# jaehyuck0103/OpenMAVIS

Measured on AMD Instinct MI355X. Metric: multi-cam frames/sec (ORB extract+match) + LocalBA iters/sec, 5x720x540, higher is better.
Workload: dtype u8

## Files before the change

### openmavis_amd/csrc/orb_extract.hip

```cpp
#include <hip/hip_runtime.h>

#include <algorithm>
#include <cmath>
#include <cstdlib>
#include <climits>
#include <cstdio>
#include <cstring>
#include <vector>

#include "../../include/omv.h"
#include "fast_plan.h"
#include "omv_device.h"
#include "omv_host.h"
#include "omv_introsort.h"

namespace {

constexpr int kMaxLevels = 16;
constexpr int kOrbStages = 4;
using omv_fast_plan::kEdge;
using omv_fast_plan::kMinB;
#define OMV_PATTERN_TABLE_BEGIN
#define OMV_PATTERN_TABLE_END
constexpr int kPattern[256 * 4] = {
#include "orb_pattern_31.inc"
};
struct FloatPattern {
    float v[256][4];
};
constexpr FloatPattern float_pattern() {
    FloatPattern p{};
    for (int i = 0; i < 256; ++i)
        for (int q = 0; q < 4; ++q) p.v[i][q] = (float)kPattern[4 * i + q];
    return p;
}
__constant__ FloatPattern c_patternf = float_pattern();
__constant__ int c_gauss7[7] = {18, 34, 48, 56, 48, 34, 18};

struct LevelGeom {
    int w, h, pitch;
    long long off;
    int maxBX, maxBY;
    int cell_begin, cell_end;
    int quota;
    int out_cap;
    int out_off;
    long long cand_off;
    int cand_cap;
    int nIni;
    float hX;
    float scale;
    float size;
    int xtab_off, ytab_off;
    int xq_off, use_xq;
    uint32_t m_quads, m_groups, m_w;
};

using omv_fast_plan::Cell;
using omv_fast_plan::FastSlot;

struct Geom {
    int nlevels;
    int W, H;
// ... 298 lines not shown

typedef _Float16 h2 __attribute__((ext_vector_type(2)));
__device__ __forceinline__ h2 h2_swap(h2 x) { return h2{x.y, x.x}; }
typedef unsigned short u16x2 __attribute__((ext_vector_type(2)));
__device__ __forceinline__ h2 h2_bytes(const uint8_t *lo, const uint8_t *hi) {
    const u16x2 v{(unsigned short)*lo, (unsigned short)*hi};
    return __builtin_bit_cast(h2, v);
}

template <int RS>
__device__ __forceinline__ int fast_strength_h(const uint8_t *p7, int stride_rt) {
    const int stride = RS > 0 ? RS : stride_rt;
    const int c = 3 * stride + 3;
    const int o[16] = {c + 3 * stride, c + 3 * stride + 1, c + 2 * stride + 2, c + stride + 3, c + 3, c - stride + 3,
                       c - 2 * stride + 2, c - 3 * stride + 1, c - 3 * stride, c - 3 * stride - 1, c - 2 * stride - 2,
                       c - stride - 3, c - 3, c + stride - 3, c + 2 * stride - 2, c + 3 * stride - 1};
    const h2 vv = h2_bytes(p7 + c, p7 + c);
    h2 d[8];
#pragma unroll
    for (int k = 0; k < 8; ++k) d[k] = vv - h2_bytes(p7 + o[k], p7 + o[k + 8]);
    auto Q = [&](const h2 *a, int k) { return k < 8 ? a[k] : h2_swap(a[k - 8]); };
    h2 t3n[8], t3x[8];
#pragma unroll
    for (int k = 0; k < 8; ++k) {
        t3n[k] = __builtin_elementwise_minimum(__builtin_elementwise_minimum(d[k], Q(d, k + 1)), Q(d, k + 2));
        t3x[k] = __builtin_elementwise_maximum(__builtin_elementwise_maximum(d[k], Q(d, k + 1)), Q(d, k + 2));
    }
    h2 a{(_Float16)-1000, (_Float16)-1000}, b{(_Float16)1000, (_Float16)1000};
#pragma unroll
    for (int k = 0; k < 8; ++k) {
        const h2 m9 = __builtin_elementwise_minimum(__builtin_elementwise_minimum(t3n[k], Q(t3n, k + 3)), Q(t3n, k + 6));
        const h2 M9 = __builtin_elementwise_maximum(__builtin_elementwise_maximum(t3x[k], Q(t3x, k + 3)), Q(t3x, k + 6));
        a = __builtin_elementwise_maximum(a, m9);
        b = __builtin_elementwise_minimum(b, M9);
    }
    const pk16 m = __builtin_elementwise_max(__builtin_bit_cast(pk16, a),
                                             __builtin_bit_cast(pk16, __builtin_bit_cast(uint32_t, b) ^ 0x80008000u));
    return max(max((int)m.x, (int)m.y), 0);
}

__device__ __forceinline__ int wave_incl_scan_dpp(int v) {
    v += __builtin_amdgcn_update_dpp(0, v, 0x111, 0xf, 0xf, false);
    v += __builtin_amdgcn_update_dpp(0, v, 0x112, 0xf, 0xf, false);
    v += __builtin_amdgcn_update_dpp(0, v, 0x114, 0xf, 0xf, false);
    v += __builtin_amdgcn_update_dpp(0, v, 0x118, 0xf, 0xf, false);
    v += __builtin_amdgcn_update_dpp(0, v, 0x142, 0xa, 0xf, false);
    v += __builtin_amdgcn_update_dpp(0, v, 0x143, 0xc, 0xf, false);
    return v;
}

#ifdef OMV_FAST_PROFILE
__device__ unsigned long long g_fast_stats[8];
#endif
template <int RS>
__global__ void __launch_bounds__(64) fast_cells_kernel(Geom g, const Cell *cells, const FastSlot *slots,
                                                        const uint8_t *images, size_t img_stride, size_t pitch0,
                                                        const uint8_t *pyr, int *cell_cnt, uint32_t *cell_kp, int rmax,
                                                        int smax, int n_blocks) {
    extern __shared__ __attribute__((aligned(16))) uint8_t smem[];
    const int blk = omv::xcd_block(n_blocks);
    if (blk < 0) return;
    const int img = blk / g.n_cells;
    const int ci = blk - img * g.n_cells;
    const Cell c = cells[ci];
    const int lane = threadIdx.x;
    const FastSlot sl0 = slots[c.slot_off + lane];
    const int rw = c.x1 - c.x0, rh = c.y1 - c.y0;
    int sp;
    const uint8_t *src = level_base(g, images, img_stride, pitch0, pyr, img, c.level, &sp);
    const uint8_t *row0 = src + (size_t)c.y0 * sp + c.x0;
    const bool dwords = ((sp & 3) == 0) && ((((uintptr_t)src) & 3) == 0);
    const int o = dwords ? c.o : 0;
    const int rs = RS > 0 ? RS : dwords ? 4 * c.nd : ((rw + 3) & ~3);
    uint8_t *pix = smem + o;
    uint8_t *S = smem + rmax;
    const int sw = rw - 4;
    uint16_t *cand = (uint16_t *)(smem + rmax + smax);
    if (dwords) {
        const int nd = c.nd;
        const uint8_t *g0 = row0 - o;
        uint32_t *l0 = (uint32_t *)smem;
        const int rpi = c.rpi, lr = omv::mul_u24(lane, (int)c.mnd) >> 16, w = lane - omv::mul_u24(lr, nd);
        if (lr < rpi) {
            uint32_t gs = (uint32_t)(omv::mul_u24(lr, sp) + 4 * w);
            uint32_t *ld = l0 + omv::mul_u24(lr, rs >> 2) + w;
            const uint32_t gstep = (uint32_t)(rpi * sp);
            const int lstep = rpi * (rs >> 2);
#pragma unroll 4
            for (int b = 0; b < c.nband; ++b, gs += gstep, ld += lstep) *ld = *(const uint32_t *)(g0 + gs);
            if (lr < rh - c.nband * rpi) *ld = *(const uint32_t *)(g0 + gs);
        }
    } else {
        for (int i = lane; i < rw * rh; i += 64) {
            const int r = i / rw, q = i - r * rw;
            pix[r * rs + q] = row0[(size_t)r * sp + q];
        }
    }
    for (int i = lane; i < (sw * (rh - 4) + 15) >> 4; i += 64) ((uint4 *)S)[i] = make_uint4(0, 0, 0, 0);
    __syncthreads();
    const int dw = rw - 6, dh = rh - 6;
    const int ndet = c.ndet;
    const uint32_t mdw = c.mdw;
    auto rowcol = [&](int i, int &r, int &q) {
        const int rr = omv::mul_u24(i, (int)mdw) >> 20;
        r = 3 + rr, q = 3 + i - omv::mul_u24(rr, dw);
    };
    const uint64_t lt = (1ull << lane) - 1ull;
#ifdef OMV_FAST_PROFILE
    int ncand_last = 0;
#endif
    auto prefilter = [&](int t) {
        int ncand = 0;
        if (dwords && ndet > 0) {
            const int rsw = rs >> 2;
            const int np = c.np;
            const pk16 T0{(short)t, (short)t};
            auto lo = [](uint32_t a, uint32_t b, uint32_t s) {
                return __builtin_bit_cast(pk16, __builtin_amdgcn_perm(a, b, 0x0c000c00u | ((s + 1) << 16) | s));
            };
            auto hi = [](uint32_t a, uint32_t b, uint32_t s) {
                return __builtin_bit_cast(pk16, __builtin_amdgcn_perm(a, b, 0x0c000c00u | ((s + 3) << 16) | (s + 2)));
            };
            auto test = [&](pk16 v, pk16 n0, pk16 n4, pk16 n8, pk16 n12) {
                const pk16 vp = v + T0, vm = v - T0;
                auto sg = [](pk16 x) { return __builtin_bit_cast(uint32_t, x); };
                const pk16 hi = __builtin_elementwise_min(__builtin_elementwise_max(n0, n8), __builtin_elementwise_max(n4, n12));
                const pk16 lo = __builtin_elementwise_max(__builtin_elementwise_min(n0, n8), __builtin_elementwise_min(n4, n12));
                return (sg(vp - hi) | sg(lo - vm)) & 0x80008000u;
            };
            auto compass = [&](uint32_t up) {
                const uint32_t *wu = reinterpret_cast<const uint32_t *>(smem + up);
                const uint32_t U0 = wu[0], U1 = wu[1];
                const uint32_t Wm = wu[3 * rsw - 1], C0 = wu[3 * rsw], C1 = wu[3 * rsw + 1], Wp = wu[3 * rsw + 2];
                const uint32_t D0 = wu[6 * rsw], D1 = wu[6 * rsw + 1];
                const uint32_t p0 = test(lo(C0, C0, 0), lo(D0, D0, 0), lo(C1, C0, 3), lo(U0, U0, 0), lo(C0, Wm, 1));
                const uint32_t p1 = test(hi(C0, C0, 0), hi(D0, D0, 0), hi(C1, C0, 3), hi(U0, U0, 0), hi(C0, Wm, 1));
                const uint32_t p2 = test(lo(C1, C1, 0), lo(D1, D1, 0), lo(Wp, C1, 3), lo(U1, U1, 0), lo(C1, C0, 1));
                const uint32_t p3 = test(hi(C1, C1, 0), hi(D1, D1, 0), hi(Wp, C1, 3), hi(U1, U1, 0), hi(C1, C0, 1));
                const uint32_t xb = (p0 >> 15) | (p1 >> 13) | (p2 >> 11) | (p3 >> 9);
                return (xb & 0x55u) | ((xb >> 15) & 0xaau);
            };
            const uint32_t lpos0 = (uint32_t)(rmax + smax);
            uint32_t lpos = lpos0;
            const uint8_t *sl = reinterpret_cast<const uint8_t *>(slots + c.slot_off);
            const uint32_t sl_lane = (uint32_t)lane * (uint32_t)sizeof(FastSlot);
            FastSlot nx = sl0;
            for (int t0 = 0; t0 < np; t0 += 64) {
                const FastSlot cur = nx;
                nx = *reinterpret_cast<const FastSlot *>(sl + (size_t)(t0 + 64) * sizeof(FastSlot) + sl_lane);
                uint32_t bits = compass(cur.hi) & (cur.lo >> 16);
                const int cnt = __popc(bits);
                const int incl = wave_incl_scan_dpp(cnt);
                if (bits) {
                    uint16_t *cp = reinterpret_cast<uint16_t *>(smem + lpos + 2u * (uint32_t)(incl - cnt)) - 1;
                    const uint32_t ebase = cur.lo & 0xffffu;
                    uint32_t below = bits - 1u;
                    for (;;) {
                        *++cp = (uint16_t)(ebase + __builtin_ctz(bits));
                        bits &= below;
                        if (__builtin_usub_overflow(bits, 1u, &below)) break;
                    }
                }
                lpos += 2u * (uint32_t)__builtin_amdgcn_readlane(incl, 63);
            }
            ncand = (int)((lpos - lpos0) >> 1);
        } else {
            for (int i0 = 0; i0 < ndet; i0 += 64) {
                const int i = i0 + lane;
                bool pass = false;
                int r = 0, q = 0;
                if (i < ndet) {
                    rowcol(i, r, q);
                    const uint8_t *p = pix + r * rs + q;
                    const int v = p[0];
                    const int d0 = v - p[3 * rs], d4 = v - p[3], d8 = v - p[-3 * rs], d12 = v - p[-3];
                    const bool a0 = d0 > t, a4 = d4 > t, a8 = d8 > t, a12 = d12 > t;
                    const bool b0 = d0 < -t, b4 = d4 < -t, b8 = d8 < -t, b12 = d12 < -t;
                    pass = (a0 && a4) || (a4 && a8) || (a8 && a12) || (a12 && a0) || (b0 && b4) || (b4 && b8) ||
                           (b8 && b12) || (b12 && b0);
                }
                const uint64_t m = __ballot(pass);
                if (pass) cand[ncand + __popcll(m & lt)] = (uint16_t)((r << 7) | q);
                ncand += __popcll(m);
            }
        }
        __syncthreads();
#ifdef OMV_FAST_PROFILE
        ncand_last = ncand;
#endif
        const uint8_t *pix7 = smem + __builtin_amdgcn_readfirstlane(o - (3 * rs + 3));
        int ncorn = 0;
        for (int k0 = 0; k0 < ncand; k0 += 64) {
            const int k = k0 + lane;
            bool corner = false;
            int e = 0;
            if (k < ncand) {
                e = cand[k];
                const int r = e >> 7, q = e & 127;
                const int sv = fast_strength_h<RS>(pix7 + r * rs + q, rs);
                S[omv::mul_u24(r - 2, sw) + (q - 2)] = (uint8_t)sv;
                corner = sv > t;
            }
            const uint64_t m = __ballot(corner);
            if (corner) cand[ncorn + __popcll(m & lt)] = (uint16_t)e;
            ncorn += __popcll(m);
        }
        __syncthreads();
        return ncorn;
    };
    auto nms = [&](int ncorn, int th, uint32_t *out) {
        int base = 0;
        for (int k0 = 0; k0 < ncorn; k0 += 64) {
            const int k = k0 + lane;
            bool keep = false;
            uint32_t packed = 0;
            if (k < ncorn) {
                const int e = cand[k];
                const int r = e >> 7, q = e & 127;
                const uint8_t *sp8 = S + omv::mul_u24(r - 2, sw) + (q - 2);
                const int v = sp8[0];
                int m = max(th, 1);
#pragma unroll
                for (int n = 0; n < 9; ++n)
                    if (n != 4) m = max(m, (int)sp8[(n / 3 - 1) * sw + (n % 3 - 1)]);
                keep = v > m;
                const int x = c.x0 + q - kMinB, y = c.y0 + r - kMinB;
                packed = (uint32_t)x | ((uint32_t)y << 12) | ((uint32_t)(v - 1) << 24);
            }
            const uint64_t m = __ballot(keep);
            const int pos = base + __popcll(m & lt);
            if (out && keep && pos < g.cell_cap) out[pos] = packed;
            base += __popcll(m);
        }
        return base;
    };
    uint32_t *out = cell_kp + (size_t)blk * g.cell_cap;
    int th = g.ini_th;
    int ncorn = prefilter(th);
#ifdef OMV_FAST_PROFILE
    const int ncand0 = ncand_last;
#endif
    int total = nms(ncorn, th, out);
    if (total == 0) {
        th = g.min_th;
        ncorn = prefilter(th);
        total = nms(ncorn, th, out);
    }
    if (lane == 0) cell_cnt[blk] = total > g.cell_cap ? -1 : total;
#ifdef OMV_FAST_PROFILE
    {
        __shared__ int dummy;
        (void)dummy;
        if (lane == 0) {
            atomicAdd(&g_fast_stats[0], 1ull);
            atomicAdd(&g_fast_stats[1], (unsigned long long)ndet);
            atomicAdd(&g_fast_stats[2], (unsigned long long)ncand0);
            atomicAdd(&g_fast_stats[3], th == g.min_th && g.min_th != g.ini_th ? 1ull : 0ull);
            atomicAdd(&g_fast_stats[4], (unsigned long long)ncand_last);
            atomicAdd(&g_fast_stats[5], (unsigned long long)total);
            atomicAdd(&g_fast_stats[6], (unsigned long long)ncorn);
            __threadfence();
            const unsigned long long done = atomicAdd(&g_fast_stats[7], 1ull) + 1;
            if (done == (unsigned long long)n_blocks)
                printf("fast: cells %llu pixels %llu cand(iniTh) %llu retries %llu cand(last pass) %llu corners(last pass) "
                       "%llu keypoints %llu\n",
                       g_fast_stats[0], g_fast_stats[1], g_fast_stats[2], g_fast_stats[3], g_fast_stats[4],
                       g_fast_stats[6], g_fast_stats[5]);
        }
    }
#endif
}

__device__ __forceinline__ int wave_incl_scan(int v) { return wave_incl_scan_dpp(v); }

__device__ int block_excl_scan(int *a, int n, int *tmp) {
    const int tid = threadIdx.x, T = blockDim.x;
    const int chunk = (n + T - 1) / T;
    const int b = min(n, tid * chunk), e = min(n, b + chunk);
    int s = 0;
    for (int i = b; i < e; ++i) s += a[i];
    const int incl = wave_incl_scan(s);
    const int wave = tid >> 6, nw = T >> 6;
    __syncthreads();
    if ((tid & 63) == 63) tmp[wave] = incl;
    __syncthreads();
    int woff = 0, tot = 0;
    for (int w = 0; w < nw; ++w) {
        if (w < wave) woff += tmp[w];
        tot += tmp[w];
    }
    int run = woff + incl - s;
    for (int i = b; i < e; ++i) {
        const int v = a[i];
        a[i] = run;
        run += v;
    }
    __syncthreads();
    return tot;
}

__device__ int2 block_excl_scan2(int *a, int na, int *b, int nb, int *tmp) {
    const int tid = threadIdx.x, T = blockDim.x;
    const int ca = (na + T - 1) / T, a0 = min(na, tid * ca), a1 = min(na, a0 + ca);
    const int cb = (nb + T - 1) / T, b0 = min(nb, tid * cb), b1 = min(nb, b0 + cb);
    int sa = 0, sb = 0;
    for (int i = a0; i < a1; ++i) sa += a[i];
    for (int i = b0; i < b1; ++i) sb += b[i];
    const int ia = wave_incl_scan(sa), ib = wave_incl_scan(sb);
    const int wave = tid >> 6, nw = T >> 6;
    __syncthreads();
    if ((tid & 63) == 63) tmp[wave] = ia, tmp[8 + wave] = ib;
    __syncthreads();
    int oa = 0, ta = 0, ob = 0, tb = 0;
    for (int w = 0; w < nw; ++w) {
        if (w < wave) oa += tmp[w], ob += tmp[8 + w];
        ta += tmp[w], tb += tmp[8 + w];
    }
    int run = oa + ia - sa;
    for (int i = a0; i < a1; ++i) {
        const int v = a[i];
        a[i] = run;
        run += v;
    }
// ... 583 lines not shown
    }
    const int rank = (int)(cl & 0x7fffffffu);
    const int row = (cl >> 31) ? total - 1 - (lap_before + rank) : mono_before + rank;
    omv_kp *kp = a.kps + (size_t)img * g.n_max + row;
    uint64_t *dst = reinterpret_cast<uint64_t *>(a.desc + ((size_t)img * g.n_max + row) * 32);
    if (lane < 4) dst[lane] = words[lane];
    if (a.harris && lane == 0) a.harris[(size_t)img * g.n_max + row] = harris;
    if (lane == 0) {
        float x = (float)cx, y = (float)cy;
        if (l != 0) x *= L.scale, y *= L.scale;
        *kp = omv_kp{x, y, L.size, angle, (float)score, l};
    }
}

inline int host_round_even(float v) { return (int)std::nearbyint(v); }

__global__ void __launch_bounds__(256) node_sort_selftest_kernel(const int *k1, const int *k2, int n, int *perm) {
    extern __shared__ __attribute__((aligned(16))) int ssm[];
    omv::SortItem *items = reinterpret_cast<omv::SortItem *>(ssm);
    omv::SortItem *tmp = items + n;
    int *LS = reinterpret_cast<int *>(tmp + n), *RS = LS + n, *stk = RS + n;
    for (int i = threadIdx.x; i < n; i += blockDim.x) items[i] = omv::SortItem{k1[i], k2[i], i};
    __syncthreads();
    omv::block_introsort_loop(items, n, stk, LS, RS, threadIdx.x, blockDim.x);
    omv::block_final_insertion_sort(items, n, tmp, threadIdx.x, blockDim.x);
    for (int i = threadIdx.x; i < n; i += blockDim.x) perm[i] = items[i].payload;
}

}

struct omv_orb {
    omv_orb_params p;
    int W, H, max_images;
    int pyr_mode = -1;
    std::vector<float> scale, inv_scale, sigma2, inv_sigma2;
    std::vector<int> quota;
    int umax[16];
    Geom g;
    Cell *d_cells = nullptr;
    FastSlot *d_slots = nullptr;
    XTab *d_xt = nullptr, *d_yt = nullptr;
    XQuad *d_xq = nullptr;
    uint32_t *d_disc = nullptr;
    uint64_t *d_bop = nullptr;
    float *harris = nullptr;
    uint8_t *d_pyr = nullptr;
    int *d_cell_cnt = nullptr;
    uint32_t *d_cell_kp = nullptr, *d_cand = nullptr, *d_nid = nullptr, *d_lvl_out = nullptr, *d_lvl_cls = nullptr;
    int *d_lvl_cnt = nullptr, *d_lap = nullptr, *d_err = nullptr;
    int rmax = 0;
    int smax = 0;
    int fast_rs = 0;
    size_t fast_lds = 0;
    size_t oct_lds = 0;
    size_t pyr_lds[kMaxLevels] = {};
    PyrBand *d_bands = nullptr;
    int pyr_nb = 0, pyr_buf_dw = 0;
    int pyr_tab_dw = 0, pyr_rows = 0;
    int pyr_ydw = 3;
    uint8_t *d_img1 = nullptr;
    omv_kp *d_kp1 = nullptr;
    uint8_t *d_desc1 = nullptr;
    int *d_n1 = nullptr;
    std::vector<int> h_lap;
    hipStream_t last_stream = nullptr;
    int last_n = 0;
    int device = 0;
    bool timing = false;
    std::vector<hipEvent_t> ev;
    double stage_ms[kOrbStages] = {};
    long long stage_calls = 0;
    omv::DeviceArena mem;
    ~omv_orb() { for (hipEvent_t e : ev) (void)hipEventDestroy(e); }
};

static void flush_timing(omv_orb *o) {
    for (size_t b = 0; b + kOrbStages + 1 <= o->ev.size(); b += kOrbStages + 1) {
        for (int k = 0; k < kOrbStages; ++k) {
            float ms = 0.f;
            (void)hipEventElapsedTime(&ms, o->ev[b + k], o->ev[b + k + 1]);
            o->stage_ms[k] += ms;
        }
        o->stage_calls++;
    }
    for (hipEvent_t e : o->ev) (void)hipEventDestroy(e);
    o->ev.clear();
}

static void mark(omv_orb *o, hipStream_t st) {
    if (!o->timing) return;
    hipEvent_t e;
    (void)hipEventCreate(&e);
    (void)hipEventRecord(e, st);
    o->ev.push_back(e);
}

static omv_status build_geometry(omv_orb *o, std::vector<Cell> &cells, std::vector<FastSlot> &slots, std::vector<XTab> &xt,
                                  std::vector<XTab> &yt, std::vector<XQuad> &xq) {
    const omv_orb_params &p = o->p;
    const int nl = p.nlevels;
    const double sf = (double)p.scale_factor;
    o->scale.assign(nl, 1.f), o->sigma2.assign(nl, 1.f), o->inv_scale.resize(nl), o->inv_sigma2.resize(nl);
    for (int i = 1; i < nl; ++i) {
        o->scale[i] = (float)(o->scale[i - 1] * sf);
        o->sigma2[i] = o->scale[i] * o->scale[i];
    }
// ... 228 lines not shown
            }
            return worst;
        };
        std::vector<PyrBand> bands;
        for (int budget : {8192, 16384}) {
            for (int nb = 8; nb <= 128 && L > 1 && !o->pyr_nb; ++nb) {
                const int worst = plan(nb, bands);
                if (worst > budget) continue;
                int tab = 0, rows = 0, ydw = 3;
                for (int l = 1; l < L; ++l) {
                    if (g.lv[l].use_xq) ydw = 4;
                    else tab = std::max(tab, 3 * g.lv[l].w);
                    for (int b = 0; b < nb; ++b) {
                        const PyrBand &pb = bands[(size_t)b * kMaxLevels + l];
                        rows = std::max(rows, pb.need_hi - pb.need_lo);
                    }
                }
                o->pyr_nb = nb, o->pyr_buf_dw = worst, o->pyr_tab_dw = (tab + 3) & ~3, o->pyr_rows = rows, o->pyr_ydw = ydw;
                if (!mem.alloc(&o->d_bands, bands.size())) return OMV_ERR_HIP;
                HIP_OK(hipMemcpy(o->d_bands, bands.data(), sizeof(PyrBand) * bands.size(), hipMemcpyHostToDevice));
                const int lds = (int)(sizeof(uint32_t) * (2 * (size_t)worst + 4 + o->pyr_tab_dw + (size_t)ydw * rows));
                if (lds > 160 * 1024) {
                    (void)mem.free(&o->d_bands);
                    o->pyr_nb = 0;
                    break;
                }
                if (lds > 64 * 1024)
                    (void)hipFuncSetAttribute((const void *)pyr_chain_kernel, hipFuncAttributeMaxDynamicSharedMemorySize, lds);
            }
        }
    }
    if (!mem.alloc(&o->d_xt, xt.size()) || !mem.alloc(&o->d_yt, yt.size())) return OMV_ERR_HIP;
    if (!xt.empty()) HIP_OK(hipMemcpy(o->d_xt, xt.data(), sizeof(XTab) * xt.size(), hipMemcpyHostToDevice));
    if (!yt.empty()) HIP_OK(hipMemcpy(o->d_yt, yt.data(), sizeof(XTab) * yt.size(), hipMemcpyHostToDevice));
    if (!mem.alloc(&o->d_xq, xq.size())) return OMV_ERR_HIP;
    if (!xq.empty()) HIP_OK(hipMemcpy(o->d_xq, xq.data(), sizeof(XQuad) * xq.size(), hipMemcpyHostToDevice));
    {
        const std::vector<uint32_t> dt = disc_table(o->umax);
        uint64_t bop[4 * 64];
        omv_fast_plan::describe_bop_table(bop);
        static_assert(64 * 8 * sizeof(uint32_t) % sizeof(uint64_t) == 0, "the operands follow the masks, 8-byte aligned");
        if (!mem.alloc(&o->d_disc, dt.size() + sizeof(bop) / sizeof(uint32_t))) return OMV_ERR_HIP;
        o->d_bop = reinterpret_cast<uint64_t *>(o->d_disc + dt.size());
        HIP_OK(hipMemcpy(o->d_disc, dt.data(), sizeof(uint32_t) * dt.size(), hipMemcpyHostToDevice));
        HIP_OK(hipMemcpy(o->d_bop, bop, sizeof(bop), hipMemcpyHostToDevice));
    }
    if (!mem.alloc(&o->d_pyr, std::max<size_t>(256, (size_t)g.pyr_bytes * n)) ||
        !mem.alloc(&o->d_cell_cnt, (size_t)g.n_cells * n) || !mem.alloc(&o->d_cell_kp, (size_t)g.n_cells * g.cell_cap * n) ||
        !mem.alloc(&o->d_cand, (size_t)g.cand_per_img * n) || !mem.alloc(&o->d_nid, (size_t)g.cand_per_img * n) ||
        !mem.alloc(&o->d_lvl_out, (size_t)g.out_per_img * n) || !mem.alloc(&o->d_lvl_cls, (size_t)g.out_per_img * n) ||
        !mem.alloc(&o->d_lvl_cnt, (size_t)3 * g.nlevels * n) || !mem.alloc(&o->d_lap, 2 * n) || !mem.alloc(&o->d_err, 1))
        return OMV_ERR_HIP;
    HIP_OK(hipMemset(o->d_err, 0, sizeof(int)));
    *out = owner.release();
    return OMV_OK;
}

omv_status omv_orb_destroy(omv_orb *o) {
    if (!o) return OMV_ERR_ARG;
    delete o;
    return OMV_OK;
}

int omv_orb_max_keypoints(const omv_orb *o) { return o ? o->g.n_max : 0; }

omv_status omv_orb_scale_tables(const omv_orb *o, float *scale, float *inv_scale, float *sigma2, float *inv_sigma2) {
    if (!o) return OMV_ERR_ARG;
    for (int l = 0; l < o->p.nlevels; ++l) {
        if (scale) scale[l] = o->scale[l];
        if (inv_scale) inv_scale[l] = o->inv_scale[l];
        if (sigma2) sigma2[l] = o->sigma2[l];
        if (inv_sigma2) inv_sigma2[l] = o->inv_sigma2[l];
    }
    return OMV_OK;
}

omv_status omv_orb_extract_batch(omv_orb *o, int n, const uint8_t *images, size_t image_stride, size_t pitch,
                                 const int *lapping, omv_kp *kps, uint8_t *desc, int *n_out, int *mono_index,
                                 void *stream) {
    if (!o || n <= 0 || n > o->max_images || !images || !lapping || !kps || !desc || !n_out || !mono_index)
        return OMV_ERR_ARG;
    if (pitch < (size_t)o->W || image_stride < pitch * o->H) return OMV_ERR_ARG;
    if (pitch >= ((size_t)1 << 24)) return OMV_ERR_ARG;
    hipStream_t st = (hipStream_t)stream;
    o->last_stream = st;
    o->last_n = n;
    const Geom &g = o->g;
    if (o->h_lap.size() < (size_t)2 * n || std::memcmp(o->h_lap.data(), lapping, sizeof(int) * 2 * n) != 0) {
        HIP_OK(hipMemcpyAsync(o->d_lap, lapping, sizeof(int) * 2 * n, hipMemcpyHostToDevice, st));
        o->h_lap.assign(lapping, lapping + 2 * n);
    }
    mark(o, st);
    const bool chain = o->pyr_mode >= 0 ? o->pyr_mode == 1 : n <= kPyrChainMaxImages;
    if (o->pyr_nb > 0 && chain) {
        const size_t lds = sizeof(uint32_t) * (2 * (size_t)o->pyr_buf_dw + 4 + o->pyr_tab_dw + (size_t)o->pyr_ydw * o->pyr_rows);
        pyr_chain_kernel<<<dim3(o->pyr_nb, n), 256, lds, st>>>(g, images, image_stride, pitch, o->d_pyr, o->d_xt, o->d_yt,
                                                               o->d_xq, o->d_bands, o->pyr_buf_dw, o->pyr_tab_dw);
    } else {
        for (int l = 1; l < g.nlevels; ++l) {
            pyr_resize_kernel<<<dim3((g.lv[l].h + kPyrBlock - 1) / kPyrBlock, n), 256, o->pyr_lds[l], st>>>(
                g, l, images, image_stride, pitch, o->d_pyr, o->d_xt, o->d_yt, o->d_xq, n);
        }
    }
    mark(o, st);
    if (o->fast_rs == 52)
        fast_cells_kernel<52><<<omv::xcd_grid(g.n_cells * n), 64, o->fast_lds, st>>>(
            g, o->d_cells, o->d_slots, images, image_stride, pitch, o->d_pyr, o->d_cell_cnt, o->d_cell_kp, o->rmax, o->smax,
            g.n_cells * n);
    else if (o->fast_rs == 68)
        fast_cells_kernel<68><<<omv::xcd_grid(g.n_cells * n), 64, o->fast_lds, st>>>(
            g, o->d_cells, o->d_slots, images, image_stride, pitch, o->d_pyr, o->d_cell_cnt, o->d_cell_kp, o->rmax, o->smax,
            g.n_cells * n);
    else
        fast_cells_kernel<0><<<omv::xcd_grid(g.n_cells * n), 64, o->fast_lds, st>>>(
            g, o->d_cells, o->d_slots, images, image_stride, pitch, o->d_pyr, o->d_cell_cnt, o->d_cell_kp, o->rmax, o->smax,
            g.n_cells * n);
    mark(o, st);
    OctArgs oa{o->d_cell_cnt, o->d_cell_kp, o->d_cand, o->d_nid, o->d_lvl_out, o->d_lvl_cls, o->d_lvl_cnt, o->d_lap, o->d_err};
    if (n <= kOctSmallImages) octree_kernel<1><<<g.nlevels * n, 256, o->oct_lds, st>>>(g, oa);
    else octree_kernel<OMV_OCT_WGS><<<g.nlevels * n, 256, o->oct_lds, st>>>(g, oa);
    mark(o, st);
    DescArgs da{images, image_stride, pitch, o->d_pyr, o->d_lvl_out, o->d_lvl_cls, o->d_lvl_cnt, kps, desc, n_out, mono_index, n,
                o->d_disc, o->harris, o->d_bop};
    const int waves = g.out_per_img * n;
    describe_kernel<<<omv::xcd_grid((waves + 3) / 4), 256, 0, st>>>(g, da, (waves + 3) / 4);
    mark(o, st);
    HIP_OK(hipGetLastError());
    return OMV_OK;
}

omv_status omv_orb_set_harris(omv_orb *o, float *harris) {
    if (!o) return OMV_ERR_ARG;
    o->harris = harris;
    return OMV_OK;
}

omv_status omv_orb_enable_timing(omv_orb *o, int on) {
    if (!o) return OMV_ERR_ARG;
    o->timing = on != 0;
    return OMV_OK;
}

omv_status omv_orb_stage_ms(omv_orb *o, double *ms4, long long *calls, int reset) {
    if (!o || !ms4) return OMV_ERR_ARG;
    HIP_OK(hipStreamSynchronize(o->last_stream));
    flush_timing(o);
    for (int k = 0; k < kOrbStages; ++k) ms4[k] = o->stage_ms[k];
    if (calls) *calls = o->stage_calls;
    if (reset) {
        for (int k = 0; k < kOrbStages; ++k) o->stage_ms[k] = 0;
        o->stage_calls = 0;
    }
    return OMV_OK;
}

omv_status omv_orb_last_error(omv_orb *o) {
    if (!o) return OMV_ERR_ARG;
    HIP_OK(hipStreamSynchronize(o->last_stream));
    int e = 0;
    HIP_OK(hipMemcpy(&e, o->d_err, sizeof(int), hipMemcpyDeviceToHost));
    HIP_OK(hipMemset(o->d_err, 0, sizeof(int)));
    return e;
}

omv_status omv_orb_extract_host(omv_orb *o, const uint8_t *image, size_t pitch, int lap0, int lap1, omv_kp *kps,
                                uint8_t *desc, int *n_out, int *mono_index) {
    if (!o || !image || !kps || !desc || !n_out || !mono_index) return OMV_ERR_ARG;
    const size_t dp = (size_t)o->W;
    if (!o->d_n1) {
// ... 61 lines not shown
```

Baseline: 53730.

## Make FAST cell kernel persistent with per-XCD atomic claims and register prefetch

Replaces the one-block-per-cell FAST launch with a persistent grid sized to occupancy. Each block claims batches of cells from per-XCD atomic counters and prefetches the next cell's pixel rows and slot data into registers while the current cell is processed. A last-block-exits counter resets the claim counters for the next launch. The intent is to hide global-load latency and cut block launch overhead, at the cost of heavy register use (up to 16 prefetch words, waves_per_eu hint), atomic contention and more complex control flow.

```diff
diff --git a/openmavis_amd/csrc/fast_claims.h b/openmavis_amd/csrc/fast_claims.h
--- /dev/null
+++ b/openmavis_amd/csrc/fast_claims.h
@@ -0,0 +1,37 @@
+#pragma once
+
+#if defined(__HIPCC__)
+#define OMV_CLAIM_FN __host__ __device__ inline
+#else
+#define OMV_CLAIM_FN inline
+#endif
+
+namespace omv_fast_claims {
+
+constexpr int kXcds = 8;
+constexpr int kCounterStride = 1024;
+constexpr int kMaxBatch = 4;
+constexpr int kExitCounter = kXcds * kCounterStride;
+constexpr int kClaimWords = kExitCounter + kCounterStride;
+
+OMV_CLAIM_FN int claim_block(int xcd, unsigned k, int j, int batch, int n) {
+    const unsigned chunk = (unsigned)(n + kXcds - 1) / kXcds;
+    const unsigned i = k * (unsigned)batch + (unsigned)j;
+    const unsigned b = (unsigned)xcd * chunk + i;
+    return (j < batch && i < chunk && b < (unsigned)n) ? (int)b : -1;
+}
+OMV_CLAIM_FN int claim_batch(int n, int grid) {
+    const int b = n / grid / 8;
+    return b < 1 ? 1 : b > kMaxBatch ? kMaxBatch : b;
+}
+OMV_CLAIM_FN unsigned first_claim(unsigned block_idx) { return block_idx / kXcds; }
+OMV_CLAIM_FN unsigned next_claim(unsigned grid, unsigned drawn) { return grid / kXcds + drawn; }
+
+OMV_CLAIM_FN int claim_grid(int resident, int n) {
+    const int cap = (n + kXcds - 1) & ~(kXcds - 1);
+    int g = resident & ~(kXcds - 1);
+    if (g < kXcds) g = kXcds;
+    return g < cap ? g : cap;
+}
+
+}
diff --git a/openmavis_amd/csrc/orb_extract.hip b/openmavis_amd/csrc/orb_extract.hip
--- a/openmavis_amd/csrc/orb_extract.hip
+++ b/openmavis_amd/csrc/orb_extract.hip
@@ -9,6 +9,7 @@
 #include <vector>
 
 #include "../../include/omv.h"
+#include "fast_claims.h"
 #include "fast_plan.h"
 #include "omv_device.h"
 #include "omv_host.h"
@@ -413,223 +414,351 @@
 #ifdef OMV_FAST_PROFILE
 __device__ unsigned long long g_fast_stats[8];
 #endif
+#ifdef OMV_FAST_PHASES
+__device__ unsigned long long g_fast_phase[7];
+#endif
+struct FastWork {
+    Cell c;
+    const uint8_t *row0;
+    int sp;
+    bool dwords;
+};
 template <int RS>
-__global__ void __launch_bounds__(64) fast_cells_kernel(Geom g, const Cell *cells, const FastSlot *slots,
-                                                        const uint8_t *images, size_t img_stride, size_t pitch0,
-                                                        const uint8_t *pyr, int *cell_cnt, uint32_t *cell_kp, int rmax,
-                                                        int smax, int n_blocks) {
+__global__ void __launch_bounds__(64) __attribute__((amdgpu_waves_per_eu(5)))
+fast_cells_kernel(Geom g, const Cell *__restrict__ cells, const FastSlot *__restrict__ slots,
+                  const uint8_t *__restrict__ images, size_t img_stride, size_t pitch0, const uint8_t *__restrict__ pyr,
+                  int *__restrict__ cell_cnt, uint32_t *__restrict__ cell_kp, int rmax, int smax, int n_blocks,
+                  unsigned *__restrict__ claims, int batch) {
+    namespace fc = omv_fast_claims;
+    constexpr int kMaxPre = RS == 52 ? 12 : 16;
     extern __shared__ __attribute__((aligned(16))) uint8_t smem[];
-    const int blk = omv::xcd_block(n_blocks);
-    if (blk < 0) return;
-    const int img = blk / g.n_cells;
-    const int ci = blk - img * g.n_cells;
-    const Cell c = cells[ci];
     const int lane = threadIdx.x;
-    const FastSlot sl0 = slots[c.slot_off + lane];
-    const int rw = c.x1 - c.x0, rh = c.y1 - c.y0;
-    int sp;
-    const uint8_t *src = level_base(g, images, img_stride, pitch0, pyr, img, c.level, &sp);
-    const uint8_t *row0 = src + (size_t)c.y0 * sp + c.x0;
-    const bool dwords = ((sp & 3) == 0) && ((((uintptr_t)src) & 3) == 0);
-    const int o = dwords ? c.o : 0;
-    const int rs = RS > 0 ? RS : dwords ? 4 * c.nd : ((rw + 3) & ~3);
-    uint8_t *pix = smem + o;
+    const int xcd = (int)(blockIdx.x & 7);
+    unsigned *ctr = claims + xcd * fc::kCounterStride;
     uint8_t *S = smem + rmax;
-    const int sw = rw - 4;
     uint16_t *cand = (uint16_t *)(smem + rmax + smax);
-    if (dwords) {
-        const int nd = c.nd;
-        const uint8_t *g0 = row0 - o;
-        uint32_t *l0 = (uint32_t *)smem;
-        const int rpi = c.rpi, lr = omv::mul_u24(lane, (int)c.mnd) >> 16, w = lane - omv::mul_u24(lr, nd);
-        if (lr < rpi) {
-            uint32_t gs = (uint32_t)(omv::mul_u24(lr, sp) + 4 * w);
-            uint32_t *ld = l0 + omv::mul_u24(lr, rs >> 2) + w;
-            const uint32_t gstep = (uint32_t)(rpi * sp);
-            const int lstep = rpi * (rs >> 2);
+    const uint64_t lt = (1ull << lane) - 1ull;
+
+    auto cell_of = [&](int b, int &img) {
+        img = __builtin_amdgcn_readfirstlane(b / g.n_cells);
+        return cells[b - img * g.n_cells];
+    };
+    auto locate = [&](FastWork &w, int img) {
+        const uint8_t *src = level_base(g, images, img_stride, pitch0, pyr, img, w.c.level, &w.sp);
+        w.row0 = src + (size_t)w.c.y0 * w.sp + w.c.x0;
+        w.dwords = ((w.sp & 3) == 0) && ((((uintptr_t)src) & 3) == 0);
+    };
+    auto band_lane = [&](const Cell &c, int &lr, int &wd) {
+        lr = omv::mul_u24(lane, (int)c.mnd) >> 16, wd = lane - omv::mul_u24(lr, c.nd);
+        return lr < c.rpi ? c.nband + (lr < (c.y1 - c.y0) - c.nband * c.rpi ? 1 : 0) : 0;
+    };
+    uint32_t pre[kMaxPre];
+#pragma unroll
+    for (int b = 0; b < kMaxPre; ++b) pre[b] = 0;
+    FastSlot nsl0{0u, 0u};
+    auto held = [&](const FastWork &w) { return w.dwords && w.c.nband < kMaxPre; };
+    auto prefetch = [&](const FastWork &w) {
+        nsl0 = slots[w.c.slot_off + lane];
+        if (!held(w)) return;
+        int lr, wd;
+        const int nb = band_lane(w.c, lr, wd);
+        const uint8_t *g0 = w.row0 - w.c.o;
+        uint32_t gs = (uint32_t)(omv::mul_u24(lr, w.sp) + 4 * wd);
+        const uint32_t gstep = (uint32_t)(w.c.rpi * w.sp);
+#pragma unroll
+        for (int b = 0; b < kMaxPre; ++b, gs += gstep) pre[b] = *(const uint32_t *)(g0 + (b < nb ? gs : 0u));
+    };
+    unsigned drawn = 0;
+    auto draw = [&]() {
+        if (lane == 0) drawn = atomicInc(ctr, 0xffffffffu);
+    };
+
+    unsigned ck = fc::first_claim(blockIdx.x);
+    int cj = 0;
+    int blk = fc::claim_block(xcd, ck, 0, batch, n_blocks);
+    FastWork nw{};
+    if (blk >= 0) {
+        int img;
+        nw.c = cell_of(blk, img);
+        locate(nw, img);
+        prefetch(nw);
+        draw();
+    }
+    while (blk >= 0) {
+#ifdef OMV_FAST_PHASES
+        const unsigned long long pt0 = wall_clock64();
+#endif
+        const FastWork cw = nw;
+        const Cell &c = cw.c;
+        const FastSlot sl0 = nsl0;
+        const int rw = c.x1 - c.x0, rh = c.y1 - c.y0;
+        const bool dwords = cw.dwords;
+        const int o = dwords ? c.o : 0;
+        const int rs = RS > 0 ? RS : dwords ? 4 * c.nd : ((rw + 3) & ~3);
+        uint8_t *pix = smem + o;
+        const int sw = rw - 4;
+        int nblk = fc::claim_block(xcd, ck, cj + 1, batch, n_blocks);
+        if (nblk >= 0) {
+            ++cj;
+        } else {
+            ck = fc::next_claim(gridDim.x, (unsigned)__builtin_amdgcn_readfirstlane((int)drawn));
+            cj = 0;
+            nblk = fc::claim_block(xcd, ck, 0, batch, n_blocks);
+        }
+        int nimg = 0;
+        if (nblk >= 0) nw.c = cell_of(nblk, nimg);
+#ifdef OMV_FAST_PHASES
+        const unsigned long long pt1 = wall_clock64() + (unsigned long long)(__builtin_amdgcn_readfirstlane((int)pre[0]) & 0);
+#endif
+        if (dwords) {
+            int lr, wd;
+            const int nb = band_lane(c, lr, wd);
+            uint32_t *ld = (uint32_t *)smem + omv::mul_u24(lr, rs >> 2) + wd;
+            const int lstep = c.rpi * (rs >> 2);
+            if (held(cw)) {
+#pragma unroll
+                for (int b = 0; b < kMaxPre; ++b, ld += lstep)
+                    if (b < nb) *ld = pre[b];
+            } else if (nb > 0) {
+                const uint8_t *g0 = cw.row0 - o;
+                uint32_t gs = (uint32_t)(omv::mul_u24(lr, cw.sp) + 4 * wd);
+                const uint32_t gstep = (uint32_t)(c.rpi * cw.sp);
 #pragma unroll 4
-            for (int b = 0; b < c.nband; ++b, gs += gstep, ld += lstep) *ld = *(const uint32_t *)(g0 + gs);
-            if (lr < rh - c.nband * rpi) *ld = *(const uint32_t *)(g0 + gs);
-        }
-    } else {
-        for (int i = lane; i < rw * rh; i += 64) {
-            const int r = i / rw, q = i - r * rw;
-            pix[r * rs + q] = row0[(size_t)r * sp + q];
-        }
-    }
-    for (int i = lane; i < (sw * (rh - 4) + 15) >> 4; i += 64) ((uint4 *)S)[i] = make_uint4(0, 0, 0, 0);
-    __syncthreads();
-    const int dw = rw - 6, dh = rh - 6;
-    const int ndet = c.ndet;
-    const uint32_t mdw = c.mdw;
-    auto rowcol = [&](int i, int &r, int &q) {
-        const int rr = omv::mul_u24(i, (int)mdw) >> 20;
-        r = 3 + rr, q = 3 + i - omv::mul_u24(rr, dw);
-    };
-    const uint64_t lt = (1ull << lane) - 1ull;
+                for (int b = 0; b < c.nband; ++b, gs += gstep, ld += lstep) *ld = *(const uint32_t *)(g0 + gs);
+                if (nb > c.nband) *ld = *(const uint32_t *)(g0 + gs);
+            }
+        } else {
+            for (int i = lane; i < rw * rh; i += 64) {
+                const int r = i / rw, q = i - r * rw;
+                pix[r * rs + q] = cw.row0[(size_t)r * cw.sp + q];
+            }
+        }
+        for (int i = lane; i < (sw * (rh - 4) + 15) >> 4; i += 64) ((uint4 *)S)[i] = make_uint4(0, 0, 0, 0);
+        __syncthreads();
+        if (nblk >= 0) locate(nw, nimg);
+#ifdef OMV_FAST_PHASES
+        const unsigned long long pt2 = wall_clock64();
+        unsigned long long pt_pre = 0, pt_str = 0;
+#endif
+        const int dw = rw - 6, dh = rh - 6;
+        const int ndet = c.ndet;
+        const uint32_t mdw = c.mdw;
+        auto rowcol = [&](int i, int &r, int &q) {
+            const int rr = omv::mul_u24(i, (int)mdw) >> 20;
+            r = 3 + rr, q = 3 + i - omv::mul_u24(rr, dw);
+        };
 #ifdef OMV_FAST_PROFILE
-    int ncand_last = 0;
-#endif
-    auto prefilter = [&](int t) {
-        int ncand = 0;
-        if (dwords && ndet > 0) {
-            const int rsw = rs >> 2;
-            const int np = c.np;
-            const pk16 T0{(short)t, (short)t};
-            auto lo = [](uint32_t a, uint32_t b, uint32_t s) {
-                return __builtin_bit_cast(pk16, __builtin_amdgcn_perm(a, b, 0x0c000c00u | ((s + 1) << 16) | s));
-            };
-            auto hi = [](uint32_t a, uint32_t b, uint32_t s) {
-                return __builtin_bit_cast(pk16, __builtin_amdgcn_perm(a, b, 0x0c000c00u | ((s + 3) << 16) | (s + 2)));
-            };
-            auto test = [&](pk16 v, pk16 n0, pk16 n4, pk16 n8, pk16 n12) {
-                const pk16 vp = v + T0, vm = v - T0;
-                auto sg = [](pk16 x) { return __builtin_bit_cast(uint32_t, x); };
-                const pk16 hi = __builtin_elementwise_min(__builtin_elementwise_max(n0, n8), __builtin_elementwise_max(n4, n12));
-                const pk16 lo = __builtin_elementwise_max(__builtin_elementwise_min(n0, n8), __builtin_elementwise_min(n4, n12));
-                return (sg(vp - hi) | sg(lo - vm)) & 0x80008000u;
-            };
-            auto compass = [&](uint32_t up) {
-                const uint32_t *wu = reinterpret_cast<const uint32_t *>(smem + up);
-                const uint32_t U0 = wu[0], U1 = wu[1];
-                const uint32_t Wm = wu[3 * rsw - 1], C0 = wu[3 * rsw], C1 = wu[3 * rsw + 1], Wp = wu[3 * rsw + 2];
-                const uint32_t D0 = wu[6 * rsw], D1 = wu[6 * rsw + 1];
-                const uint32_t p0 = test(lo(C0, C0, 0), lo(D0, D0, 0), lo(C1, C0, 3), lo(U0, U0, 0), lo(C0, Wm, 1));
-                const uint32_t p1 = test(hi(C0, C0, 0), hi(D0, D0, 0), hi(C1, C0, 3), hi(U0, U0, 0), hi(C0, Wm, 1));
-                const uint32_t p2 = test(lo(C1, C1, 0), lo(D1, D1, 0), lo(Wp, C1, 3), lo(U1, U1, 0), lo(C1, C0, 1));
-                const uint32_t p3 = test(hi(C1, C1, 0), hi(D1, D1, 0), hi(Wp, C1, 3), hi(U1, U1, 0), hi(C1, C0, 1));
-                const uint32_t xb = (p0 >> 15) | (p1 >> 13) | (p2 >> 11) | (p3 >> 9);
-                return (xb & 0x55u) | ((xb >> 15) & 0xaau);
-            };
-            const uint32_t lpos0 = (uint32_t)(rmax + smax);
-            uint32_t lpos = lpos0;
-            const uint8_t *sl = reinterpret_cast<const uint8_t *>(slots + c.slot_off);
-            const uint32_t sl_lane = (uint32_t)lane * (uint32_t)sizeof(FastSlot);
-            FastSlot nx = sl0;
-            for (int t0 = 0; t0 < np; t0 += 64) {
-                const FastSlot cur = nx;
-                nx = *reinterpret_cast<const FastSlot *>(sl + (size_t)(t0 + 64) * sizeof(FastSlot) + sl_lane);
-                uint32_t bits = compass(cur.hi) & (cur.lo >> 16);
-                const int cnt = __popc(bits);
-                const int incl = wave_incl_scan_dpp(cnt);
-                if (bits) {
-                    uint16_t *cp = reinterpret_cast<uint16_t *>(smem + lpos + 2u * (uint32_t)(incl - cnt)) - 1;
-                    const uint32_t ebase = cur.lo & 0xffffu;
-                    uint32_t below = bits - 1u;
-                    for (;;) {
-                        *++cp = (uint16_t)(ebase + __builtin_ctz(bits));
-                        bits &= below;
-                        if (__builtin_usub_overflow(bits, 1u, &below)) break;
+        int ncand_last = 0;
+#endif
+        auto compass_pass = [&](int t) {
+#ifdef OMV_FAST_PHASES
+            const unsigned long long ptb = wall_clock64();
+#endif
+            int ncand = 0;
+            if (dwords && ndet > 0) {
+                const int rsw = rs >> 2;
+                const int np = c.np;
+                const pk16 T0{(short)t, (short)t};
+                auto lo = [](uint32_t a, uint32_t b, uint32_t s) {
+                    return __builtin_bit_cast(pk16, __builtin_amdgcn_perm(a, b, 0x0c000c00u | ((s + 1) << 16) | s));
+                };
+                auto hi = [](uint32_t a, uint32_t b, uint32_t s) {
+                    return __builtin_bit_cast(pk16, __builtin_amdgcn_perm(a, b, 0x0c000c00u | ((s + 3) << 16) | (s + 2)));
+                };
+                auto test = [&](pk16 v, pk16 n0, pk16 n4, pk16 n8, pk16 n12) {
+                    const pk16 vp = v + T0, vm = v - T0;
+                    auto sg = [](pk16 x) { return __builtin_bit_cast(uint32_t, x); };
+                    const pk16 hi = __builtin_elementwise_min(__builtin_elementwise_max(n0, n8), __builtin_elementwise_max(n4, n12));
+                    const pk16 lo = __builtin_elementwise_max(__builtin_elementwise_min(n0, n8), __builtin_elementwise_min(n4, n12));
+                    return (sg(vp - hi) | sg(lo - vm)) & 0x80008000u;
+                };
+                auto compass = [&](uint32_t up) {
+                    const uint32_t *wu = reinterpret_cast<const uint32_t *>(smem + up);
+                    const uint32_t U0 = wu[0], U1 = wu[1];
+                    const uint32_t Wm = wu[3 * rsw - 1], C0 = wu[3 * rsw], C1 = wu[3 * rsw + 1], Wp = wu[3 * rsw + 2];
+                    const uint32_t D0 = wu[6 * rsw], D1 = wu[6 * rsw + 1];
+                    const uint32_t p0 = test(lo(C0, C0, 0), lo(D0, D0, 0), lo(C1, C0, 3), lo(U0, U0, 0), lo(C0, Wm, 1));
+                    const uint32_t p1 = test(hi(C0, C0, 0), hi(D0, D0, 0), hi(C1, C0, 3), hi(U0, U0, 0), hi(C0, Wm, 1));
+                    const uint32_t p2 = test(lo(C1, C1, 0), lo(D1, D1, 0), lo(Wp, C1, 3), lo(U1, U1, 0), lo(C1, C0, 1));
+                    const uint32_t p3 = test(hi(C1, C1, 0), hi(D1, D1, 0), hi(Wp, C1, 3), hi(U1, U1, 0), hi(C1, C0, 1));
+                    const uint32_t xb = (p0 >> 15) | (p1 >> 13) | (p2 >> 11) | (p3 >> 9);
+                    return (xb & 0x55u) | ((xb >> 15) & 0xaau);
+                };
+                const uint32_t lpos0 = (uint32_t)(rmax + smax);
+                uint32_t lpos = lpos0;
+                const uint8_t *sl = reinterpret_cast<const uint8_t *>(slots + c.slot_off);
+                const uint32_t sl_lane = (uint32_t)lane * (uint32_t)sizeof(FastSlot);
+                FastSlot nx = sl0;
+                for (int t0 = 0; t0 < np; t0 += 64) {
+                    const FastSlot cur = nx;
+                    nx = *reinterpret_cast<const FastSlot *>(sl + (size_t)(t0 + 64) * sizeof(FastSlot) + sl_lane);
+                    uint32_t bits = compass(cur.hi) & (cur.lo >> 16);
+                    const int cnt = __popc(bits);
+                    const int incl = wave_incl_scan_dpp(cnt);
+                    if (bits) {
+                        uint16_t *cp = reinterpret_cast<uint16_t *>(smem + lpos + 2u * (uint32_t)(incl - cnt)) - 1;
+                        const uint32_t ebase = cur.lo & 0xffffu;
+                        uint32_t below = bits - 1u;
+                        for (;;) {
+                            *++cp = (uint16_t)(ebase + __builtin_ctz(bits));
+                            bits &= below;
+                            if (__builtin_usub_overflow(bits, 1u, &below)) break;
+                        }
                     }
+                    lpos += 2u * (uint32_t)__builtin_amdgcn_readlane(incl, 63);
                 }
-                lpos += 2u * (uint32_t)__builtin_amdgcn_readlane(incl, 63);
-            }
-            ncand = (int)((lpos - lpos0) >> 1);
-        } else {
-            for (int i0 = 0; i0 < ndet; i0 += 64) {
-                const int i = i0 + lane;
-                bool pass = false;
-                int r = 0, q = 0;
-                if (i < ndet) {
-                    rowcol(i, r, q);
-                    const uint8_t *p = pix + r * rs + q;
-                    const int v = p[0];
-                    const int d0 = v - p[3 * rs], d4 = v - p[3], d8 = v - p[-3 * rs], d12 = v - p[-3];
-                    const bool a0 = d0 > t, a4 = d4 > t, a8 = d8 > t, a12 = d12 > t;
-                    const bool b0 = d0 < -t, b4 = d4 < -t, b8 = d8 < -t, b12 = d12 < -t;
-                    pass = (a0 && a4) || (a4 && a8) || (a8 && a12) || (a12 && a0) || (b0 && b4) || (b4 && b8) ||
-                           (b8 && b12) || (b12 && b0);
+                asm volatile("" ::"v"(nx.lo), "v"(nx.hi));
+                ncand = (int)((lpos - lpos0) >> 1);
+            } else {
+                for (int i0 = 0; i0 < ndet; i0 += 64) {
+                    const int i = i0 + lane;
+                    bool pass = false;
+                    int r = 0, q = 0;
+                    if (i < ndet) {
+                        rowcol(i, r, q);
+                        const uint8_t *p = pix + r * rs + q;
+                        const int v = p[0];
+                        const int d0 = v - p[3 * rs], d4 = v - p[3], d8 = v - p[-3 * rs], d12 = v - p[-3];
+                        const bool a0 = d0 > t, a4 = d4 > t, a8 = d8 > t, a12 = d12 > t;
+                        const bool b0 = d0 < -t, b4 = d4 < -t, b8 = d8 < -t, b12 = d12 < -t;
+                        pass = (a0 && a4) || (a4 && a8) || (a8 && a12) || (a12 && a0) || (b0 && b4) || (b4 && b8) ||
+                               (b8 && b12) || (b12 && b0);
+                    }
+                    const uint64_t m = __ballot(pass);
+                    if (pass) cand[ncand + __popcll(m & lt)] = (uint16_t)((r << 7) | q);
+                    ncand += __popcll(m);
                 }
-                const uint64_t m = __ballot(pass);
-                if (pass) cand[ncand + __popcll(m & lt)] = (uint16_t)((r << 7) | q);
-                ncand += __popcll(m);
-            }
-        }
-        __syncthreads();
+            }
+            __syncthreads();
+#ifdef OMV_FAST_PHASES
+            pt_pre += wall_clock64() - ptb;
+#endif
+            return ncand;
+        };
+        auto strength_pass = [&](int t, int ncand) {
+#ifdef OMV_FAST_PHASES
+            const unsigned long long pta = wall_clock64();
+#endif
 #ifdef OMV_FAST_PROFILE
-        ncand_last = ncand;
-#endif
-        const uint8_t *pix7 = smem + __builtin_amdgcn_readfirstlane(o - (3 * rs + 3));
-        int ncorn = 0;
-        for (int k0 = 0; k0 < ncand; k0 += 64) {
-            const int k = k0 + lane;
-            bool corner = false;
-            int e = 0;
-            if (k < ncand) {
-                e = cand[k];
-                const int r = e >> 7, q = e & 127;
-                const int sv = fast_strength_h<RS>(pix7 + r * rs + q, rs);
-                S[omv::mul_u24(r - 2, sw) + (q - 2)] = (uint8_t)sv;
-                corner = sv > t;
-            }
-            const uint64_t m = __ballot(corner);
-            if (corner) cand[ncorn + __popcll(m & lt)] = (uint16_t)e;
-            ncorn += __popcll(m);
-        }
-        __syncthreads();
-        return ncorn;
-    };
-    auto nms = [&](int ncorn, int th, uint32_t *out) {
-        int base = 0;
-        for (int k0 = 0; k0 < ncorn; k0 += 64) {
-            const int k = k0 + lane;
-            bool keep = false;
-            uint32_t packed = 0;
-            if (k < ncorn) {
-                const int e = cand[k];
-                const int r = e >> 7, q = e & 127;
-                const uint8_t *sp8 = S + omv::mul_u24(r - 2, sw) + (q - 2);
-                const int v = sp8[0];
-                int m = max(th, 1);
-#pragma unroll
-                for (int n = 0; n < 9; ++n)
-                    if (n != 4) m = max(m, (int)sp8[(n / 3 - 1) * sw + (n % 3 - 1)]);
-                keep = v > m;
-                const int x = c.x0 + q - kMinB, y = c.y0 + r - kMinB;
-                packed = (uint32_t)x | ((uint32_t)y << 12) | ((uint32_t)(v - 1) << 24);
-            }
-            const uint64_t m = __ballot(keep);
-            const int pos = base + __popcll(m & lt);
-            if (out && keep && pos < g.cell_cap) out[pos] = packed;
-            base += __popcll(m);
-        }
-        return base;
-    };
-    uint32_t *out = cell_kp + (size_t)blk * g.cell_cap;
-    int th = g.ini_th;
-    int ncorn = prefilter(th);
+            ncand_last = ncand;
+#endif
+            const uint8_t *pix7 = smem + __builtin_amdgcn_readfirstlane(o - (3 * rs + 3));
+            int ncorn = 0;
+            for (int k0 = 0; k0 < ncand; k0 += 64) {
+                const int k = k0 + lane;
+                bool corner = false;
+                int e = 0;
+                if (k < ncand) {
+                    e = cand[k];
+                    const int r = e >> 7, q = e & 127;
+                    const int sv = fast_strength_h<RS>(pix7 + r * rs + q, rs);
+                    S[omv::mul_u24(r - 2, sw) + (q - 2)] = (uint8_t)sv;
+                    corner = sv > t;
+                }
+                const uint64_t m = __ballot(corner);
+                if (corner) cand[ncorn + __popcll(m & lt)] = (uint16_t)e;
+                ncorn += __popcll(m);
+            }
+            __syncthreads();
+#ifdef OMV_FAST_PHASES
+            pt_str += wall_clock64() - pta;
+#endif
+            return ncorn;
+        };
+        auto nms = [&](int ncorn, int th, uint32_t *out) {
+            int base = 0;
+            for (int k0 = 0; k0 < ncorn; k0 += 64) {
+                const int k = k0 + lane;
+                bool keep = false;
+                uint32_t packed = 0;
+                if (k < ncorn) {
+                    const int e = cand[k];
+                    const int r = e >> 7, q = e & 127;
+                    const uint8_t *sp8 = S + omv::mul_u24(r - 2, sw) + (q - 2);
+                    const int v = sp8[0];
+                    int m = max(th, 1);
+#pragma unroll
+                    for (int n = 0; n < 9; ++n)
+                        if (n != 4) m = max(m, (int)sp8[(n / 3 - 1) * sw + (n % 3 - 1)]);
+                    keep = v > m;
+                    const int x = c.x0 + q - kMinB, y = c.y0 + r - kMinB;
+                    packed = (uint32_t)x | ((uint32_t)y << 12) | ((uint32_t)(v - 1) << 24);
+                }
+                const uint64_t m = __ballot(keep);
+                const int pos = base + __popcll(m & lt);
+                if (out && keep && pos < g.cell_cap) out[pos] = packed;
+                base += __popcll(m);
+            }
+            return base;
+        };
+        uint32_t *out = cell_kp + (size_t)blk * g.cell_cap;
+        int th = g.ini_th;
+        int ncand = compass_pass(th);
+        if (nblk >= 0) {
+            prefetch(nw);
+            if (cj == 0) draw();
+        }
+        int ncorn = strength_pass(th, ncand);
 #ifdef OMV_FAST_PROFILE
-    const int ncand0 = ncand_last;
-#endif
-    int total = nms(ncorn, th, out);
-    if (total == 0) {
-        th = g.min_th;
-        ncorn = prefilter(th);
-        total = nms(ncorn, th, out);
-    }
-    if (lane == 0) cell_cnt[blk] = total > g.cell_cap ? -1 : total;
+        const int ncand0 = ncand_last;
+#endif
+        int total = nms(ncorn, th, out);
+        if (total == 0) {
+            th = g.min_th;
+            ncorn = strength_pass(th, compass_pass(th));
+            total = nms(ncorn, th, out);
+        }
+        if (lane == 0) cell_cnt[blk] = total > g.cell_cap ? -1 : total;
 #ifdef OMV_FAST_PROFILE
-    {
-        __shared__ int dummy;
-        (void)dummy;
-        if (lane == 0) {
-            atomicAdd(&g_fast_stats[0], 1ull);
-            atomicAdd(&g_fast_stats[1], (unsigned long long)ndet);
-            atomicAdd(&g_fast_stats[2], (unsigned long long)ncand0);
-            atomicAdd(&g_fast_stats[3], th == g.min_th && g.min_th != g.ini_th ? 1ull : 0ull);
-            atomicAdd(&g_fast_stats[4], (unsigned long long)ncand_last);
-            atomicAdd(&g_fast_stats[5], (unsigned long long)total);
-            atomicAdd(&g_fast_stats[6], (unsigned long long)ncorn);
+        {
+            __shared__ int dummy;
+            (void)dummy;
+            if (lane == 0) {
+                atomicAdd(&g_fast_stats[0], 1ull);
+                atomicAdd(&g_fast_stats[1], (unsigned long long)ndet);
+                atomicAdd(&g_fast_stats[2], (unsigned long long)ncand0);
+                atomicAdd(&g_fast_stats[3], th == g.min_th && g.min_th != g.ini_th ? 1ull : 0ull);
+                atomicAdd(&g_fast_stats[4], (unsigned long long)ncand_last);
+                atomicAdd(&g_fast_stats[5], (unsigned long long)total);
+                atomicAdd(&g_fast_stats[6], (unsigned long long)ncorn);
+                __threadfence();
+                const unsigned long long done = atomicAdd(&g_fast_stats[7], 1ull) + 1;
+                if (done == (unsigned long long)n_blocks)
+                    printf("fast: cells %llu pixels %llu cand(iniTh) %llu retries %llu cand(last pass) %llu corners(last pass) "
+                           "%llu keypoints %llu\n",
+                           g_fast_stats[0], g_fast_stats[1], g_fast_stats[2], g_fast_stats[3], g_fast_stats[4],
+                           g_fast_stats[6], g_fast_stats[5]);
+            }
+        }
+#endif
+#ifdef OMV_FAST_PHASES
+        if (lane == 0 && (blk & 63) == 0) {
+            const unsigned long long pt3 = wall_clock64();
+            atomicAdd(&g_fast_phase[0], pt1 - pt0);
+            atomicAdd(&g_fast_phase[1], pt2 - pt1);
+            atomicAdd(&g_fast_phase[2], pt_pre);
+            atomicAdd(&g_fast_phase[3], pt_str);
+            atomicAdd(&g_fast_phase[4], pt3 - pt2 - pt_pre - pt_str);
+            atomicAdd(&g_fast_phase[5], pt3 - pt0);
             __threadfence();
-            const unsigned long long done = atomicAdd(&g_fast_stats[7], 1ull) + 1;
-            if (done == (unsigned long long)n_blocks)
-                printf("fast: cells %llu pixels %llu cand(iniTh) %llu retries %llu cand(last pass) %llu corners(last pass) "
-                       "%llu keypoints %llu\n",
-                       g_fast_stats[0], g_fast_stats[1], g_fast_stats[2], g_fast_stats[3], g_fast_stats[4],
-                       g_fast_stats[6], g_fast_stats[5]);
-        }
-    }
-#endif
+            const unsigned long long cnt = (unsigned long long)((n_blocks + 63) >> 6);
+            const unsigned long long done = atomicAdd(&g_fast_phase[6], 1ull) + 1;
+            if (done % cnt == 0)
+                printf("fast phases, 10 ns ticks summed over %llu sampled cells: preamble %llu staging %llu compass %llu "
+                       "strength %llu nms %llu life %llu\n",
+                       done, g_fast_phase[0], g_fast_phase[1], g_fast_phase[2], g_fast_phase[3], g_fast_phase[4], g_fast_phase[5]);
+        }
+#endif
+        blk = nblk;
+    }
+    if (lane == 0) {
+        unsigned *gone = claims + fc::kExitCounter;
+        if (__hip_atomic_fetch_add(gone, 1u, __ATOMIC_RELAXED, __HIP_MEMORY_SCOPE_AGENT) + 1u == gridDim.x) {
+            for (int x = 0; x < fc::kXcds; ++x)
+                __hip_atomic_store(claims + x * fc::kCounterStride, 0u, __ATOMIC_RELAXED, __HIP_MEMORY_SCOPE_AGENT);
+            __hip_atomic_store(gone, 0u, __ATOMIC_RELAXED, __HIP_MEMORY_SCOPE_AGENT);
+        }
+    }
 }
 
 __device__ __forceinline__ int wave_incl_scan(int v) { return wave_incl_scan_dpp(v); }
@@ -1319,6 +1448,9 @@
     int smax = 0;
     int fast_rs = 0;
     size_t fast_lds = 0;
+    int fast_wgs = 0;
+    int fast_batch = 0;
+    unsigned *d_claims = nullptr;
     size_t oct_lds = 0;
     size_t pyr_lds[kMaxLevels] = {};
     PyrBand *d_bands = nullptr;
@@ -1653,6 +1785,22 @@
         !mem.alloc(&o->d_lvl_cnt, (size_t)3 * g.nlevels * n) || !mem.alloc(&o->d_lap, 2 * n) || !mem.alloc(&o->d_err, 1))
         return OMV_ERR_HIP;
     HIP_OK(hipMemset(o->d_err, 0, sizeof(int)));
+    {
+        const void *fn = o->fast_rs == 52   ? (const void *)fast_cells_kernel<52>
+                         : o->fast_rs == 68 ? (const void *)fast_cells_kernel<68>
+                                            : (const void *)fast_cells_kernel<0>;
+        int per_cu = 0, cus = 0;
+        HIP_OK(hipOccupancyMaxActiveBlocksPerMultiprocessor(&per_cu, fn, 64, o->fast_lds));
+        HIP_OK(hipDeviceGetAttribute(&cus, hipDeviceAttributeMultiprocessorCount, o->device));
+        if (per_cu < 1 || cus < 1) return OMV_ERR_HIP;
+        o->fast_wgs = per_cu * cus;
+        if (const char *e = getenv("OMV_FAST_WGS"))
+            if (std::atoi(e) > 0) o->fast_wgs = std::atoi(e);
+        if (const char *e = getenv("OMV_FAST_BATCH")) o->fast_batch = std::min(std::max(std::atoi(e), 0), omv_fast_claims::kMaxBatch);
+        const std::vector<unsigned> zero(omv_fast_claims::kClaimWords, 0u);
+        if (!mem.alloc(&o->d_claims, zero.size())) return OMV_ERR_HIP;
+        HIP_OK(hipMemcpy(o->d_claims, zero.data(), sizeof(unsigned) * zero.size(), hipMemcpyHostToDevice));
+    }
     *out = owner.release();
     return OMV_OK;
 }
@@ -1704,18 +1852,20 @@
         }
     }
     mark(o, st);
+    const int fast_grid = omv_fast_claims::claim_grid(o->fast_wgs, g.n_cells * n);
+    const int fast_batch = o->fast_batch > 0 ? o->fast_batch : omv_fast_claims::claim_batch(g.n_cells * n, fast_grid);
     if (o->fast_rs == 52)
-        fast_cells_kernel<52><<<omv::xcd_grid(g.n_cells * n), 64, o->fast_lds, st>>>(
-            g, o->d_cells, o->d_slots, images, image_stride, pitch, o->d_pyr, o->d_cell_cnt, o->d_cell_kp, o->rmax, o->smax,
-            g.n_cells * n);
+        fast_cells_kernel<52><<<fast_grid, 64, o->fast_lds, st>>>(g, o->d_cells, o->d_slots, images, image_stride, pitch,
+                                                                  o->d_pyr, o->d_cell_cnt, o->d_cell_kp, o->rmax, o->smax,
+                                                                  g.n_cells * n, o->d_claims, fast_batch);
     else if (o->fast_rs == 68)
-        fast_cells_kernel<68><<<omv::xcd_grid(g.n_cells * n), 64, o->fast_lds, st>>>(
-            g, o->d_cells, o->d_slots, images, image_stride, pitch, o->d_pyr, o->d_cell_cnt, o->d_cell_kp, o->rmax, o->smax,
-            g.n_cells * n);
+        fast_cells_kernel<68><<<fast_grid, 64, o->fast_lds, st>>>(g, o->d_cells, o->d_slots, images, image_stride, pitch,
+                                                                  o->d_pyr, o->d_cell_cnt, o->d_cell_kp, o->rmax, o->smax,
+                                                                  g.n_cells * n, o->d_claims, fast_batch);
     else
-        fast_cells_kernel<0><<<omv::xcd_grid(g.n_cells * n), 64, o->fast_lds, st>>>(
-            g, o->d_cells, o->d_slots, images, image_stride, pitch, o->d_pyr, o->d_cell_cnt, o->d_cell_kp, o->rmax, o->smax,
-            g.n_cells * n);
+        fast_cells_kernel<0><<<fast_grid, 64, o->fast_lds, st>>>(g, o->d_cells, o->d_slots, images, image_stride, pitch,
+                                                                 o->d_pyr, o->d_cell_cnt, o->d_cell_kp, o->rmax, o->smax,
+                                                                 g.n_cells * n, o->d_claims, fast_batch);
     mark(o, st);
     OctArgs oa{o->d_cell_cnt, o->d_cell_kp, o->d_cand, o->d_nid, o->d_lvl_out, o->d_lvl_cls, o->d_lvl_cnt, o->d_lap, o->d_err};
     if (n <= kOctSmallImages) octree_kernel<1><<<g.nlevels * n, 256, o->oct_lds, st>>>(g, oa);
```

Result: slower. 52670 (-2.0%).
